# MyrtleSoftware/myrtlespeech

Measured on AMD Instinct MI355X. Metric: audio-sec/s (RTF), DS2 5xBiLSTM-1024 encoder forward + CTC greedy, 80-feature 10 s clips @ batch 32/GPU, higher is better.
Workload: dtype f16x3 (f32 split in fp16 hi+lo, 3 fp16 MFMA passes, f32 acc: LSTM, projections, conv1/2, FC1; FC2/CTC/decode f32)

## Files before the change

include/ms_hotpath.h:

```cpp
#ifndef MS_HOTPATH_H
#define MS_HOTPATH_H

#include <stddef.h>
#include <stdint.h>

#ifdef __cplusplus
extern "C" {
#endif

#define MS_ABI_VERSION 4

enum {
  MS_OK = 0,
  MS_ERR_INVALID = 1,
  MS_ERR_HIP = 2,
  MS_ERR_WORKSPACE = 3,
  MS_ERR_TIMEOUT = 4,
  MS_ERR_UNSUPPORTED = 5
};

enum { MS_CELL_LSTM = 0, MS_CELL_GRU = 1, MS_CELL_RNN_TANH = 2, MS_CELL_HARD_LSTM = 3 };

enum { MS_ACT_NONE = 0, MS_ACT_CLAMP = 1  };

int ms_abi_version(void);
const char* ms_last_error(void);


int ms_mask_time_(float* x, const int32_t* lens, int N, int inner, int T, void* stream);

size_t ms_maskconv_packed_bytes(int Cout, int Cin_g, int KF, int KT, int groups);

int ms_maskconv_pack(const float* w, void* packed, int Cout, int Cin_g, int KF, int KT, int groups, void* stream);

int ms_maskconv_forward(const float* x, const int32_t* lens, const void* packed_w, const float* bias, float* y,
                        int N, int Cin, int Fin, int Tin, int Cout, int Fout, int Tout, int KF, int KT, int SF,
                        int ST, int DF, int DT, int pad_f_l, int pad_t_l, int groups, int act, float act_lo,
                        float act_hi, void* stream);

size_t ms_maskconv_cl_packed_bytes(int Cout, int Cin, int KF, int KT);
int ms_maskconv_cl_pack(const float* w, void* packed, int Cout, int Cin, int KF, int KT, void* stream);
size_t ms_maskconv_cl_workspace_bytes(int N, int Cin, int Fin, int Tin);
int ms_maskconv_cl_forward(const float* x, const int32_t* lens, const void* packed_w, const float* bias, float* y,
                           int N, int Cin, int Fin, int Tin, int Cout, int Fout, int Tout, int KF, int KT, int SF,
                           int ST, int DF, int DT, int pad_f_l, int pad_t_l, int act, float act_lo, float act_hi,
                           void* workspace, size_t workspace_bytes, void* stream);

size_t ms_maskconv_fwin_packed_bytes(int Cout, int KF, int KT);
int ms_maskconv_fwin_pack(const float* w, void* packed, int Cout, int KF, int KT, void* stream);
size_t ms_maskconv_fwin_workspace_bytes(int N, int Tin, int KF, int SF, int Fout);
int ms_maskconv_fwin_forward(const float* x, const int32_t* lens, const void* packed_w, const float* bias, float* y, int N,
                             int Fin, int Tin, int Cout, int Fout, int Tout, int KF, int KT, int SF, int ST, int DT,
                             int pad_f_l, int pad_t_l, int act, float act_lo, float act_hi, void* workspace,
                             size_t workspace_bytes, void* stream);

int ms_maskconv_fwin_planes_supported(int N, int Tin, int Cout, int Fout, int Tout, int KF, int KT, int SF, int ST, int DT);
int ms_maskconv_cl_supported(int N, int Cin, int Fin, int Cout, int Fout, int Tout, int KT, int ST, int DT);
int ms_maskconv_fwin_planes_forward(const float* x, const int32_t* lens, const void* packed_w, const float* bias, void* planes,
                                    size_t planes_bytes, int N, int Fin, int Tin, int Cout, int Fout, int Tout, int KF, int KT,
                                    int SF, int ST, int DT, int pad_f_l, int pad_t_l, int act, float act_lo, float act_hi,
                                    void* workspace, size_t workspace_bytes, void* stream);
int ms_maskconv_cl_planes_forward(const int32_t* lens, const void* packed_w, const float* bias, float* y, int N, int Cin,
                                  int Fin, int Tin, int Cout, int Fout, int Tout, int KF, int KT, int SF, int ST, int DF,
                                  int DT, int pad_f_l, int pad_t_l, int act, float act_lo, float act_hi, void* planes,
                                  size_t planes_bytes, void* stream);

int ms_conv_set_variant(int variant);

size_t ms_maskconv1d_gemm_packed_bytes(int Cout, int Cin, int KT);
int ms_maskconv1d_gemm_pack(const float* w, void* packed, int Cout, int Cin, int KT, void* stream);
size_t ms_maskconv1d_gemm_workspace_bytes(int N, int Cin, int Tout, int Cout, int KT);
int ms_maskconv1d_gemm_forward(const float* x, const int32_t* lens, const void* packed, const float* bias, float* y, int N,
                               int Cin, int Tin, int Cout, int Tout, int KT, int ST, int DT, int pad_l, int act,
                               float act_lo, float act_hi, void* workspace, size_t workspace_bytes, void* stream);

int ms_nct_to_tnc(const float* x, float* y, int N, int CF, int T, void* stream);

int ms_clamp(const float* x, float* y, size_t n, float lo, float hi, void* stream);


int ms_linear_forward(const float* x, const float* w, const float* bias, float* y, int M, int K, int N, int act,
                      float act_lo, float act_hi, void* stream);

#define MS_LINEAR_FEW_ROWS 1
size_t ms_linear_splitk_workspace_bytes(int M, int K, int N, int flags);
int ms_linear_splitk_forward(const float* x, const float* w, const float* bias, float* y, int M, int K, int N, int act,
                             float act_lo, float act_hi, int flags, void* workspace, size_t workspace_bytes, void* stream);

size_t ms_linear_split_workspace_bytes(int M, int K, int N);
int ms_linear_split_forward(const float* x, const float* w, const float* bias, float* y, int M, int K, int N, int act,
                            float act_lo, float act_hi, void* workspace, size_t workspace_bytes, void* stream);

size_t ms_linear_split_packed_bytes(int K, int N);
int ms_linear_split_pack(const float* w, void* packed, int K, int N, void* stream);
int ms_linear_split_forward_packed(const float* x, const void* packed_w, const float* bias, float* y, int M, int K, int N, int act,
                                   float act_lo, float act_hi, void* workspace, size_t workspace_bytes, void* stream);


int ms_lookahead_forward(const float* x, const float* w, float* y, int N, int F, int T, int ctx, long xs_n,
                         long xs_f, long xs_t, long ys_n, long ys_f, long ys_t, int act, float act_lo,
                         float act_hi, void* stream);

int ms_lookahead_window_forward(const float* x, const float* w, float* y, int N, int F, int T_in, int T_out, int ctx,
                                long xs_n, long xs_f, long xs_t, long ys_n, long ys_f, long ys_t, int act, float act_lo,
                                float act_hi, void* stream);


int ms_rnn_padded_hidden(int cell, int H, int ndir);
size_t ms_rnn_packed_bytes(int cell, int In, int H, int ndir);
int ms_rnn_pack(int cell, int In, int H, int ndir, const float* const* w_ih_host, const float* const* w_hh_host,
                const float* const* b_ih_host, const float* const* b_hh_host, void* packed, void* stream);

size_t ms_rnn_workspace_bytes(int cell, int T, int N, int In, int H, int ndir);

int ms_rnn_layer_forward(int cell, const void* packed, const float* x, const int32_t* lens, int max_len,
                         const float* h0, const float* c0, float* out, float* hn, float* cn, int T, int N, int In,
                         int H, int ndir, void* workspace, size_t workspace_bytes, void* stream);

enum { MS_RNN_X_PLANES_IN_WS = 1, MS_RNN_OUT_PLANES_TO_WS = 2, MS_RNN_PACKED_ROWS = 4, MS_RNN_HX_PREINIT = 4096,
       MS_RNN_RECURRENCE_ONLY = 8192, MS_RNN_TIMING_SKIP_PROJECTION = 8192 ,
// ... 258 lines not shown
```

myrtlespeech_amd/_lib.py:

```python
import ctypes
import os
import re
from ctypes import POINTER, c_char_p, c_double, c_float, c_int, c_int32, c_int64, c_long, c_size_t, c_uint64, c_void_p

import torch

_HERE = os.path.dirname(os.path.abspath(__file__))
LIB_PATH = os.environ.get("MS_HOTPATH_LIB") or os.path.join(_HERE, "libms_hotpath.so")
HEADER_PATH = os.path.join(os.path.dirname(_HERE), "include", "ms_hotpath.h")

MS_OK = 0
ABI_VERSION = 4
ERR_NAMES = {1: "MS_ERR_INVALID", 2: "MS_ERR_HIP", 3: "MS_ERR_WORKSPACE", 4: "MS_ERR_TIMEOUT", 5: "MS_ERR_UNSUPPORTED"}

CELL_LSTM, CELL_GRU, CELL_RNN_TANH, CELL_HARD_LSTM = 0, 1, 2, 3
ACT_NONE, ACT_CLAMP = 0, 1
LINEAR_FEW_ROWS = 1
PROF_KINDS = 9

_P = c_void_p
_PP = POINTER(c_void_p)

SIGNATURES = {
    "ms_abi_version": (c_int, []),
    "ms_last_error": (c_char_p, []),
    "ms_mask_time_": (c_int, [_P, _P, c_int, c_int, c_int, _P]),
    "ms_maskconv_packed_bytes": (c_size_t, [c_int, c_int, c_int, c_int, c_int]),
    "ms_maskconv_pack": (c_int, [_P, _P, c_int, c_int, c_int, c_int, c_int, _P]),
    "ms_maskconv_forward": (c_int, [_P, _P, _P, _P, _P] + [c_int] * 17 + [c_float, c_float, _P]),
    "ms_maskconv_cl_packed_bytes": (c_size_t, [c_int, c_int, c_int, c_int]),
    "ms_maskconv_cl_pack": (c_int, [_P, _P, c_int, c_int, c_int, c_int, _P]),
    "ms_maskconv_cl_workspace_bytes": (c_size_t, [c_int, c_int, c_int, c_int]),
    "ms_maskconv_cl_forward": (c_int, [_P, _P, _P, _P, _P] + [c_int] * 16 + [c_float, c_float, _P, c_size_t, _P]),
    "ms_maskconv_fwin_packed_bytes": (c_size_t, [c_int, c_int, c_int]),
    "ms_maskconv_fwin_pack": (c_int, [_P, _P, c_int, c_int, c_int, _P]),
    "ms_maskconv_fwin_workspace_bytes": (c_size_t, [c_int, c_int, c_int, c_int, c_int]),
    "ms_maskconv_fwin_forward": (c_int, [_P, _P, _P, _P, _P] + [c_int] * 14 + [c_float, c_float, _P, c_size_t, _P]),
    "ms_maskconv_fwin_planes_forward": (c_int, [_P, _P, _P, _P, _P, c_size_t] + [c_int] * 14 + [c_float, c_float, _P, c_size_t, _P]),
    "ms_maskconv_cl_planes_forward": (c_int, [_P, _P, _P, _P] + [c_int] * 16 + [c_float, c_float, _P, c_size_t, _P]),
    "ms_maskconv_fwin_planes_supported": (c_int, [c_int] * 10),
    "ms_maskconv_cl_supported": (c_int, [c_int] * 9),
    "ms_conv_set_variant": (c_int, [c_int]),
    "ms_maskconv1d_gemm_packed_bytes": (c_size_t, [c_int, c_int, c_int]),
    "ms_maskconv1d_gemm_pack": (c_int, [_P, _P, c_int, c_int, c_int, _P]),
    "ms_maskconv1d_gemm_workspace_bytes": (c_size_t, [c_int] * 5),
    "ms_maskconv1d_gemm_forward": (c_int, [_P, _P, _P, _P, _P] + [c_int] * 10 + [c_float, c_float, _P, c_size_t, _P]),
    "ms_nct_to_tnc": (c_int, [_P, _P, c_int, c_int, c_int, _P]),
    "ms_clamp": (c_int, [_P, _P, c_size_t, c_float, c_float, _P]),
    "ms_linear_forward": (c_int, [_P, _P, _P, _P, c_int, c_int, c_int, c_int, c_float, c_float, _P]),
    "ms_linear_splitk_workspace_bytes": (c_size_t, [c_int, c_int, c_int, c_int]),
    "ms_linear_splitk_forward": (c_int, [_P, _P, _P, _P, c_int, c_int, c_int, c_int, c_float, c_float, c_int, _P, c_size_t, _P]),
    "ms_linear_split_workspace_bytes": (c_size_t, [c_int, c_int, c_int]),
    "ms_linear_split_forward": (c_int, [_P, _P, _P, _P, c_int, c_int, c_int, c_int, c_float, c_float, _P, c_size_t, _P]),
    "ms_linear_split_packed_bytes": (c_size_t, [c_int, c_int]),
    "ms_linear_split_pack": (c_int, [_P, _P, c_int, c_int, _P]),
    "ms_linear_split_forward_packed": (c_int, [_P, _P, _P, _P, c_int, c_int, c_int, c_int, c_float, c_float, _P, c_size_t, _P]),
    "ms_lookahead_forward": (c_int, [_P, _P, _P, c_int, c_int, c_int, c_int] + [c_long] * 6 + [c_int, c_float, c_float, _P]),
    "ms_lookahead_window_forward": (c_int, [_P, _P, _P, c_int, c_int, c_int, c_int, c_int] + [c_long] * 6 + [c_int, c_float, c_float, _P]),
    "ms_rnn_packed_bytes": (c_size_t, [c_int, c_int, c_int, c_int]),
    "ms_ctc_status": (c_int, [_P, _P]),
    "ms_rnn_padded_hidden": (c_int, [c_int, c_int, c_int]),
    "ms_rnn_hx_preinit": (c_int, [c_int] * 8 + [_P, c_size_t, _P]),
    "ms_rnn_pack": (c_int, [c_int, c_int, c_int, c_int, _PP, _PP, _PP, _PP, _P, _P]),
    "ms_rnn_workspace_bytes": (c_size_t, [c_int] * 6),
    "ms_rnn_layer_forward": (c_int, [c_int, _P, _P, _P, c_int, _P, _P, _P, _P, _P] + [c_int] * 5 + [_P, c_size_t, _P]),
    "ms_rnn_layer_forward_ex": (c_int, [c_int, _P, _P, _P, c_int, _P, _P, _P, _P, _P] + [c_int] * 6 + [_P, c_size_t, _P]),
    "ms_rnn_layer_chains_planes": (c_int, [c_int, c_int, c_int]),
    "ms_rnn_layer_is_wide": (c_int, [c_int] * 4),
    "ms_rnn_stack_overlap_ok": (c_int, [c_int] * 7),
    "ms_rnn_stack_forward": (c_int, [c_int, _P, _P, _P, c_int, _P, _P, _P, _P, _P] + [c_int] * 7 + [_P, c_size_t, _P]),
    "ms_rnn_status": (c_int, [_P, _P]),
    "ms_rnn_debug_offset": (c_size_t, [c_int] * 6),
    "ms_rnn_layer_packs_rows": (c_int, [c_int] * 6),
    "ms_gemm_set_variant": (c_int, [c_int]),
    "ms_prof_enable": (c_int, [c_int]),
    "ms_prof_read": (c_int, [POINTER(c_float), POINTER(c_int)]),
    "ms_clock_probe": (c_int, [_P, c_int, c_int, _P]),
    "ms_barrier_chain_probe": (c_int, [_P, c_int, c_int, _P]),
    "ms_ctc_loss_workspace_bytes": (c_size_t, [c_int] * 4),
    "ms_ctc_loss_forward": (c_int, [_P] * 7 + [c_int] * 7 + [_P, c_size_t, _P]),
    "ms_log_softmax_axis": (c_int, [_P, _P, c_int, c_int, c_int, _P]),
    "ms_log_softmax_axis_backward": (c_int, [_P, _P, _P, c_int, c_int, c_int, _P]),
    "ms_ctc_loss_backward_workspace_bytes": (c_size_t, [c_int] * 4),
    "ms_ctc_loss_backward": (c_int, [_P] * 7 + [c_int] * 6 + [_P, c_size_t, _P]),
    "ms_ctc_greedy_decode": (c_int, [_P, _P, _P, _P, c_int, c_int, c_int, c_int, _P]),
    "ms_ctc_align_workspace_bytes": (c_size_t, [c_int] * 4),
    "ms_ctc_align": (c_int, [_P] * 10 + [c_int] * 6 + [_P, c_size_t, _P]),
    "ms_ctc_greedy_stream_state_bytes": (c_size_t, [c_int]),
    "ms_ctc_greedy_stream_begin": (c_int, [_P, c_int, _P]),
    "ms_ctc_greedy_stream_step": (c_int, [_P, c_int, c_int, c_int, c_int, _P, _P, _P, _P, c_int, _P, _P, c_int, _P]),
    "ms_embedding_forward": (c_int, [_P, _P, _P, c_int, c_int, c_int, _P]),
    "ms_rnnt_joint_forward": (c_int, [_P, _P, _P, _P, _P, _P, c_int, c_int, c_int, _P]),
    "ms_rnnt_topk": (c_int, [_P, _P, _P, c_int, c_int, c_int, _P]),
    "ms_ctc_beam_workspace_bytes": (c_size_t, [c_int] * 4),
# ... 266 lines not shown
```

myrtlespeech_amd/csrc/api_common.cpp:

```cpp
#include <cstdlib>
#include <cstring>
#include <mutex>
#include <vector>

#include <algorithm>
#include "common.h"

namespace ms {
static thread_local std::string g_err;
void set_error(const std::string& s) { g_err = s; }
int num_cus() {
  static std::atomic<int> cus[64];
  int dev = 0;
  if (hipGetDevice(&dev) != hipSuccess) return 0;
  int v = cus[dev & 63].load(std::memory_order_relaxed);
  if (v == 0) {
    hipDeviceProp_t p;
    if (hipGetDeviceProperties(&p, dev) != hipSuccess) return 0;
    v = p.multiProcessorCount;
    cus[dev & 63].store(v, std::memory_order_relaxed);
  }
  return v;
}
int precision_mode() {
  static int v = -1;
  if (v < 0) {
    const char* e = getenv("MS_PRECISION");
    v = PREC_F16X3;
    if (e && strcmp(e, "f32") == 0) v = PREC_F32;
    if (e && strcmp(e, "fp16") == 0) v = PREC_F16;
    if (e && strcmp(e, "bf16x3") == 0) v = PREC_BF16X3;
  }
  return v;
}

namespace {
__global__ void absmax_bits_kernel(const float* __restrict__ w, size_t n, unsigned* __restrict__ out) {
  unsigned m = 0;
  for (size_t i = (size_t)blockIdx.x * blockDim.x + threadIdx.x; i < n; i += (size_t)gridDim.x * blockDim.x) {
    const unsigned b = __float_as_uint(w[i]) & 0x7FFFFFFFu;
    if (b < 0x7F800000u) m = max(m, b);
  }
  for (int o = 32; o > 0; o >>= 1) m = max(m, (unsigned)__shfl_xor((int)m, o, 64));
  if ((threadIdx.x & 63) == 0 && m) atomicMax(out, m);
}
__global__ void scale_word_kernel(float* __restrict__ word, int half_planes) {
  const unsigned bits = __float_as_uint(word[0]);
  int s = 0;
  if (half_planes && bits != 0) {
    const int e = (int)((bits >> 23) & 255) - 127;
    s = min(max(12 - e, -100), 100);
  }
  word[0] = ldexpf(1.0f, s);
  word[1] = ldexpf(1.0f, -s);
}
}

int weight_scale_launch(const float* w, size_t n, float* scale_word, int prec, hipStream_t stream) {
  MS_HIP(hipMemsetAsync(scale_word, 0, 2 * sizeof(float), stream));
  const bool half_planes = prec == PREC_F16X3 || prec == PREC_F16;
  if (half_planes && n > 0) {
    const int blocks = (int)std::min<size_t>((n + 255) / 256, 1024);
    hipLaunchKernelGGL(absmax_bits_kernel, dim3(blocks), dim3(256), 0, stream, w, n, (unsigned*)scale_word);
  }
  hipLaunchKernelGGL(scale_word_kernel, dim3(1), dim3(1), 0, stream, scale_word, half_planes ? 1 : 0);
  MS_LAUNCH_CHECK();
  return MS_OK;
}

namespace {
struct ProfSpan { hipEvent_t a, b; int kind; };
std::atomic<bool> g_prof_on{false};
std::mutex g_prof_mu;
std::vector<ProfSpan> g_spans;
std::vector<ProfSpan> g_free;
}

ProfScope::ProfScope(int kind_, hipStream_t st) : kind(kind_), stream(st), on(g_prof_on.load(std::memory_order_relaxed)) {
  if (!on) return;
  {
    std::lock_guard<std::mutex> lk(g_prof_mu);
    if (!g_free.empty()) { a = g_free.back().a; b = g_free.back().b; g_free.pop_back(); }
  }
  if (!a && (hipEventCreate(&a) != hipSuccess || hipEventCreate(&b) != hipSuccess)) { on = false; return; }
  (void)hipEventRecord(a, stream);
}
ProfScope::~ProfScope() {
  if (!on) return;
  (void)hipEventRecord(b, stream);
  std::lock_guard<std::mutex> lk(g_prof_mu);
  g_spans.push_back({a, b, kind});
}
}

extern "C" int ms_prof_enable(int on) {
  ms::g_prof_on.store(on != 0, std::memory_order_relaxed);
  return MS_OK;
}

extern "C" int ms_prof_read(float* out_ms, int* out_n) {
  MS_REQUIRE(out_ms && out_n, "null pointer");
  for (int k = 0; k < MS_PROF_KINDS; ++k) { out_ms[k] = 0.f; out_n[k] = 0; }
  std::lock_guard<std::mutex> lk(ms::g_prof_mu);
  for (auto& s : ms::g_spans) {
    MS_HIP(hipEventSynchronize(s.b));
    float t = 0.f;
    MS_HIP(hipEventElapsedTime(&t, s.a, s.b));
    if (s.kind >= 0 && s.kind < MS_PROF_KINDS) { out_ms[s.kind] += t; out_n[s.kind] += 1; }
    ms::g_free.push_back(s);
  }
  ms::g_spans.clear();
  return MS_OK;
}

// ... 57 lines not shown
```

myrtlespeech_amd/csrc/conv_cl.hip:

```cpp
#include <algorithm>
#include <type_traits>

#include "common.h"

namespace {

typedef unsigned u32x4 __attribute__((ext_vector_type(4)));
typedef unsigned u32x2 __attribute__((ext_vector_type(2)));
typedef __bf16 bf16x8 __attribute__((ext_vector_type(8)));
typedef _Float16 f16x8 __attribute__((ext_vector_type(8)));

constexpr int CL_F = 2;

struct ClP {
  int N, Cin, Fin, Tin, Cout, Fout, Tout, KF, KT, SF, ST, DF, DT, pad_f, pad_t;
  int KG;
  int KW;
  int PW;
  int co_tiles;
  int act;
  float lo, hi;
  int FP;
  int CS, RG, SG, PQ;
};
// ... 256 lines not shown
  };
  constexpr std::integral_constant<int, 0> S0{};
  constexpr std::integral_constant<int, 1> S1{};
  if (wave < p.KF) load_row(S0, wave);
  for (int kf = wave; kf < p.KF; kf += 8) {
    if (kf + 4 < p.KF) load_row(S1, kf + 4);
    compute_row(S0, kf);
    if (kf + 8 < p.KF) load_row(S0, kf + 8);
    if (kf + 4 < p.KF) compute_row(S1, kf + 4);
  }

  __syncthreads();
  ms::f32x4* part = reinterpret_cast<ms::f32x4*>(lds);
#pragma unroll
  for (int i = 0; i < SH_RB; ++i)
    if (i < RB) part[(wave * SH_RB + i) * 64 + lane] = acc[i];
  __syncthreads();
#pragma unroll
  for (int j = 0; j < SH_RB / 4; ++j) {
    const int i = wave + 4 * j, fo = fo0 + i;
    if (i >= RB || fo >= p.Fout) continue;
    ms::f32x4 v = part[(0 * SH_RB + i) * 64 + lane];
#pragma unroll
    for (int w = 1; w < 4; ++w) v += part[(w * SH_RB + i) * 64 + lane];
    if (c16 < p.Tout) {
#pragma unroll
      for (int r = 0; r < 4; ++r) {
        const int co = cb * 16 + 4 * q + r;
        if (co < p.Cout) {
          float o = v[r] * winv + (bias ? bias[co] : 0.f);
          if (p.act == MS_ACT_CLAMP) o = ms::act_clamp(o, p.lo, p.hi);
          y[(((size_t)n * p.Cout + co) * p.Fout + fo) * p.Tout + c16] = o;
        }
      }
    }
  }
}

int conv_cl_short_plan(const ClP& p, bool f16, int* RB, int* RIN, size_t* lds) {
  static const bool off = getenv("MS_CONV_SHORT") && getenv("MS_CONV_SHORT")[0] == '0';
  if (off || p.Cin != 32 || p.Tout > 16 || p.ST != 1 || p.DT != 1 || p.FP != 0 || p.N > 65535 || p.KT > SH_KT) return 0;
  const int cbs = ms::cdiv(p.Cout, 16);
  int nblk = std::max(1, std::min(ms::cdiv(p.Fout, 4), ms::cdiv(ms::num_cus(), p.N * cbs)));
  while (ms::cdiv(p.Fout, nblk) > SH_RB) ++nblk;
  for (; nblk <= p.Fout; ++nblk) {
    const int rb = ms::cdiv(p.Fout, nblk);
    const int rin = (rb - 1) * p.SF + (p.KF - 1) * p.DF + 1;
    const size_t bytes = std::max((size_t)(f16 ? 1 : 2) * rin * (p.Tout + p.KT - 1) * 64, (size_t)4 * SH_RB * 64 * 16);
    if (bytes <= 156 * 1024) { *RB = rb; *RIN = rin; *lds = bytes; return 1; }
  }
  return 0;
}

constexpr int FS_TT = 64;
constexpr int FS_MR = 5;
constexpr int FS_TS = 2;
constexpr int FS_PF = 2;

template <int P>
__global__ __launch_bounds__(256, 2) void maskconv_fwin_shared_kernel(const unsigned short* __restrict__ xh,
                                                                      const unsigned short* __restrict__ xl,
                                                                      const int32_t* __restrict__ lens,
                                                                      const unsigned short* __restrict__ wp,
                                                                      const float* __restrict__ bias, float* __restrict__ y,
                                                                      unsigned short* __restrict__ oh,
                                                                      unsigned short* __restrict__ ol, ClP p,
                                                                      const float* __restrict__ scale_word) {
  constexpr bool F16 = ms::prec_one_plane(P), HM = P == ms::PREC_F16X3;
  extern __shared__ __attribute__((aligned(16))) char lds[];
  const int gran_bytes = p.ST * p.PQ * 16;
  const int in_plane = p.SG * gran_bytes;
  char* Ph = lds;
  char* Pl = lds + in_plane;
  char* Wh = lds + (F16 ? 1 : 2) * in_plane;
  char* Wl = Wh + FS_TS * p.KG * 32 * 16;

  const int tid = threadIdx.x, lane = tid & 63, wave = tid >> 6;
  const int l31 = lane & 31, half = lane >> 5;
  const int fb = wave & 1, rg = wave >> 1;
  const int t0 = blockIdx.x * FS_TT;
  const int cls = blockIdx.y % p.CS, jb = blockIdx.y / p.CS;
  const int fo_first = cls + jb * (2 * FS_MR) * p.CS;
  if (fo_first >= p.Fout) return;
  const int nrows = min(2 * FS_MR, (p.Fout - 1 - fo_first) / p.CS + 1);
  const int n = blockIdx.z / p.co_tiles, tile = blockIdx.z % p.co_tiles;
  const int len = lens ? min(lens[n], p.Tin) : p.Tin;
  const int cout_pad = p.co_tiles * 32;
  const size_t wplane = (size_t)p.KT * p.KG * cout_pad * 8;

  u32x4 fh[FS_PF], fl[FS_PF];
  auto load_filters = [&](int kt0) {
    const int ng = min(FS_TS, p.KT - kt0) * p.KG * 32;
#pragma unroll
    for (int j = 0; j < FS_PF; ++j) {
      const int i = tid + 256 * j;
      if (i < ng) {
        const int co = i & 31, rest = i >> 5;
        const size_t src = (((size_t)kt0 * p.KG + rest) * cout_pad + tile * 32 + co) * 8;
        fh[j] = *reinterpret_cast<const u32x4*>(wp + src);
        if (!F16) fl[j] = *reinterpret_cast<const u32x4*>(wp + wplane + src);
      }
    }
  };
  auto store_filters = [&](int kt0) {
    const int ng = min(FS_TS, p.KT - kt0) * p.KG * 32;
#pragma unroll
// ... 74 lines not shown
          }
        }
      };
      for (int s = 0; s < s_full; ++s) k_step(s, std::false_type{});
      if (s_full < p.KG / 2) k_step(s_full, std::true_type{});
    }
    if (more) {
      __syncthreads();
      store_filters(kt0 + FS_TS);
      __syncthreads();
    }
  }

  const int t = t0 + fb * 32 + l31;
  const float winv = scale_word[1];
  if (t < p.Tout) {
#pragma unroll
    for (int f = 0; f < FS_MR; ++f) {
      const int j = rg * FS_MR + f;
      if (j >= nrows) continue;
      const int fo = fo_first + j * p.CS;
      if (oh) {
#pragma unroll
        for (int r4 = 0; r4 < 4; ++r4) {
          const int co = tile * 32 + ms::mfma32_row(4 * r4, lane);
          if (co >= p.Cout) continue;
          unsigned h[4], l[4];
#pragma unroll
          for (int e = 0; e < 4; ++e) {
            float v = acc[f][4 * r4 + e] * winv + (bias ? bias[co + e] : 0.f);
            if (p.act == MS_ACT_CLAMP) v = ms::act_clamp(v, p.lo, p.hi);
            split_act_by_prec(v, P, h[e], l[e]);
          }
          const size_t o = (((size_t)n * p.Fout + fo) * p.Tout + t) * p.Cout + co;
          *reinterpret_cast<u32x2*>(oh + o) = u32x2{h[0] | (h[1] << 16), h[2] | (h[3] << 16)};
          if (!F16) *reinterpret_cast<u32x2*>(ol + o) = u32x2{l[0] | (l[1] << 16), l[2] | (l[3] << 16)};
        }
        continue;
      }
#pragma unroll
      for (int r = 0; r < 16; ++r) {
        const int co = tile * 32 + ms::mfma32_row(r, lane);
        if (co < p.Cout) {
          float v = acc[f][r] * winv + (bias ? bias[co] : 0.f);
          if (p.act == MS_ACT_CLAMP) v = ms::act_clamp(v, p.lo, p.hi);
          y[(((size_t)n * p.Cout + co) * p.Fout + fo) * p.Tout + t] = v;
        }
      }
    }
  }
}

int conv_fs_plan(ClP& p, bool f16, size_t* lds) {
  if (g_conv_variant.load(std::memory_order_relaxed) != 0 || p.Tout <= 48 || p.SF % 2) return 0;
  int g = 2 * p.SF, b = 16;
  while (b) { const int r = g % b; g = b; b = r; }
  p.CS = 16 / g;
  p.RG = p.CS * p.SF / 8;
  p.SG = (2 * FS_MR - 1) * p.RG + p.KG;
  p.PW = (FS_TT - 1) * p.ST + (p.KT - 1) * p.DT + 1;
  p.PQ = ms::cdiv(p.PW, p.ST);
  const int planes = f16 ? 1 : 2;
  *lds = (size_t)planes * ((size_t)p.SG * p.ST * p.PQ * 16 + (size_t)FS_TS * p.KG * 32 * 16);
  const long rows_y = (long)p.CS * ms::cdiv(ms::cdiv(p.Fout, p.CS), 2 * FS_MR);
  if (p.SG > 16 || FS_TS * p.KG * 32 > 256 * FS_PF || *lds > 160 * 1024 || rows_y > 65535 || (long)p.N * p.co_tiles > 65535)
    return 0;
  return 1;
}

int conv_fs_launch(const ClP& p, size_t lds, const unsigned short* xh, const unsigned short* xl, const int32_t* lens,
                   const void* packed_w, const float* bias, float* y, unsigned short* oh, unsigned short* ol,
                   hipStream_t stream, const float* scale_word) {
  static ms::DeviceOnce attr_once;
  if (attr_once.need()) {
    MS_HIP(hipFuncSetAttribute((const void*)maskconv_fwin_shared_kernel<ms::PREC_BF16X3>, hipFuncAttributeMaxDynamicSharedMemorySize, 160 * 1024));
    MS_HIP(hipFuncSetAttribute((const void*)maskconv_fwin_shared_kernel<ms::PREC_F16>, hipFuncAttributeMaxDynamicSharedMemorySize, 160 * 1024));
    MS_HIP(hipFuncSetAttribute((const void*)maskconv_fwin_shared_kernel<ms::PREC_F16X3>, hipFuncAttributeMaxDynamicSharedMemorySize, 160 * 1024));
    attr_once.done();
  }
  const int prec = ms::split_mode();
  const dim3 grid(ms::cdiv(p.Tout, FS_TT), p.CS * ms::cdiv(ms::cdiv(p.Fout, p.CS), 2 * FS_MR), p.N * p.co_tiles);
  const unsigned short* wq = (const unsigned short*)packed_w;
  auto kern = prec == ms::PREC_F16 ? maskconv_fwin_shared_kernel<ms::PREC_F16>
              : prec == ms::PREC_F16X3 ? maskconv_fwin_shared_kernel<ms::PREC_F16X3> : maskconv_fwin_shared_kernel<ms::PREC_BF16X3>;
  hipLaunchKernelGGL(kern, grid, dim3(256), lds, stream, xh, xl, lens, wq, bias, y, oh, ol, p, scale_word);
  MS_LAUNCH_CHECK();
  return MS_OK;
}

__global__ void nchw_to_cl_split_kernel(const float* __restrict__ x, unsigned short* __restrict__ hi,
                                        unsigned short* __restrict__ lo, int C, int F, int T, int prec) {
  __shared__ float tile[32][33];
  const int n = blockIdx.z / F, f = blockIdx.z % F;
  const int t0 = blockIdx.x * 32, c0 = blockIdx.y * 32;
  const int tx = threadIdx.x, ty = threadIdx.y;
  for (int i = ty; i < 32; i += 8) {
    const int c = c0 + i, t = t0 + tx;
    tile[i][tx] = (c < C && t < T) ? x[(((size_t)n * C + c) * F + f) * T + t] : 0.f;
  }
  __syncthreads();
  for (int i = ty; i < 32; i += 8) {
    const int t = t0 + i, c = c0 + tx;
    if (t < T && c < C) {
      const float v = tile[tx][i];
      const size_t o = (((size_t)n * F + f) * T + t) * C + c;
      unsigned h, l;
      split_act_by_prec(v, prec, h, l);
// ... 201 lines not shown
  MS_REQUIRE(planes, "null pointer");
  MS_REQUIRE(Cout > 0 && Cout % 16 == 0, "planes out need Cout % 16 == 0 (the next convolution's k-steps)");
  if (N <= 0 || Fout <= 0 || Tout <= 0 || planes_bytes < ms_maskconv_cl_workspace_bytes(N, Cout, Fout, Tout)) {
    ms::set_error("ms_maskconv_fwin_planes_forward: planes buffer too small");
    return MS_ERR_WORKSPACE;
  }
  return fwin_forward(x, lens, packed_w, bias, nullptr, planes, N, Fin, Tin, Cout, Fout, Tout, KF, KT, SF, ST, DT, pad_f_l,
                      pad_t_l, act, act_lo, act_hi, workspace, workspace_bytes, stream_);
}

extern "C" int ms_conv_set_variant(int v) {
  g_conv_variant.store(v, std::memory_order_relaxed);
  return MS_OK;
}

static size_t cl_plane_bytes(int Cout, int Cin, int KF, int KT) {
  return ms::align_up((size_t)2 * KF * KT * (Cin / 8) * (ms::cdiv(Cout, 32) * 32) * 8 * sizeof(unsigned short), 256);
}
extern "C" size_t ms_maskconv_cl_packed_bytes(int Cout, int Cin, int KF, int KT) {
  if (Cout <= 0 || Cin <= 0 || Cin % 16 || KF <= 0 || KT <= 0) return 0;
  return cl_plane_bytes(Cout, Cin, KF, KT) + 256;
}

extern "C" int ms_maskconv_cl_pack(const float* w, void* packed, int Cout, int Cin, int KF, int KT, void* stream) {
  MS_REQUIRE(w && packed, "null pointer");
  MS_REQUIRE(Cout > 0 && Cin > 0 && Cin % 16 == 0 && KF > 0 && KT > 0, "bad shape (Cin must be a multiple of 16)");
  const int cout_pad = ms::cdiv(Cout, 32) * 32;
  const size_t plane = (size_t)KF * KT * (Cin / 8) * cout_pad * 8;
  const int blocks = (int)std::min<size_t>((plane + 255) / 256, 2048);
  float* scale_word = (float*)((char*)packed + cl_plane_bytes(Cout, Cin, KF, KT));
  const int rc = ms::weight_scale_launch(w, (size_t)Cout * Cin * KF * KT, scale_word, ms::split_mode(), (hipStream_t)stream);
  if (rc != MS_OK) return rc;
  hipLaunchKernelGGL(conv_cl_pack_kernel, dim3(blocks), dim3(256), 0, (hipStream_t)stream, w, (unsigned short*)packed, Cout,
                     Cin, KF, KT, cout_pad, ms::split_mode(), scale_word);
  MS_LAUNCH_CHECK();
  return MS_OK;
}

extern "C" size_t ms_maskconv_cl_workspace_bytes(int N, int Cin, int Fin, int Tin) {
  if (N <= 0 || Cin <= 0 || Fin <= 0 || Tin <= 0) return 0;
  return ms::align_up((size_t)N * Cin * Fin * Tin * 4, 256);
}

extern "C" int ms_maskconv_cl_supported(int N, int Cin, int Fin, int Cout, int Fout, int Tout, int KT, int ST, int DT) {
  if (N <= 0 || Cin <= 0 || Cin % 16 || Fin <= 0 || Cout <= 0 || Fout <= 0 || Tout <= 0 || KT <= 0 || ST <= 0 || DT <= 0 ||
      (long)N * Fin > 65535)
    return 0;
  ClP p{};
  p.N = N; p.Fout = Fout; p.Tout = Tout; p.KT = KT; p.ST = ST; p.DT = DT; p.KG = Cin / 8; p.co_tiles = ms::cdiv(Cout, 32);
  size_t lds = 0;
  return conv_cl_plan(p, &lds) != 0;
}

static int cl_forward(const float* x, const int32_t* lens, const void* packed_w, const float* bias, float* y,
                      int N, int Cin, int Fin, int Tin, int Cout, int Fout, int Tout, int KF, int KT,
                      int SF, int ST, int DF, int DT, int pad_f_l, int pad_t_l, int act, float act_lo,
                      float act_hi, void* workspace, size_t workspace_bytes, void* stream_) {
  ms::ProfScope prof_span(MS_PROF_CONV, (hipStream_t)stream_);
  MS_REQUIRE(packed_w && y && workspace, "null pointer");
  MS_REQUIRE(N > 0 && Cin > 0 && Cin % 16 == 0 && Fin > 0 && Tin > 0 && Cout > 0 && Fout > 0 && Tout > 0, "bad shape");
  MS_REQUIRE(KF > 0 && KT > 0 && SF > 0 && ST > 0 && DF > 0 && DT > 0 && pad_f_l >= 0 && pad_t_l >= 0, "bad kernel");
  MS_REQUIRE(act == MS_ACT_NONE || act == MS_ACT_CLAMP, "bad act");
  if (workspace_bytes < ms_maskconv_cl_workspace_bytes(N, Cin, Fin, Tin)) {
    ms::set_error("ms_maskconv_cl_forward: workspace too small");
    return MS_ERR_WORKSPACE;
  }
  hipStream_t stream = (hipStream_t)stream_;
  ClP p;
  p.N = N; p.Cin = Cin; p.Fin = Fin; p.Tin = Tin; p.Cout = Cout; p.Fout = Fout; p.Tout = Tout; p.KF = KF; p.KT = KT;
  p.SF = SF; p.ST = ST; p.DF = DF; p.DT = DT; p.pad_f = pad_f_l; p.pad_t = pad_t_l; p.KG = Cin / 8;
  p.co_tiles = ms::cdiv(Cout, 32);
  p.act = act; p.lo = act_lo; p.hi = act_hi;
  p.FP = 0;
  p.KW = 0;
  p.CS = p.RG = p.SG = p.PQ = 0;
  size_t lds = 0;
  const int wf = conv_cl_plan(p, &lds);
  if (wf == 0) {
    ms::set_error("ms_maskconv_cl_forward: shape outside the LDS / grid budget");
    return MS_ERR_UNSUPPORTED;
  }
  const float* scale_word = (const float*)((const char*)packed_w + cl_plane_bytes(Cout, Cin, KF, KT));
  unsigned short* xh = (unsigned short*)workspace;
  unsigned short* xl = xh + (size_t)N * Cin * Fin * Tin;
  MS_REQUIRE(N * Fin <= 65535, "N*Fin exceeds grid limits");
  const int prec = ms::split_mode();
  const bool f16 = prec == ms::PREC_F16;
  if (x) {
    hipLaunchKernelGGL(nchw_to_cl_split_kernel, dim3(ms::cdiv(Tin, 32), ms::cdiv(Cin, 32), N * Fin), dim3(32, 8), 0, stream, x,
                       xh, xl, Cin, Fin, Tin, prec);
    MS_LAUNCH_CHECK();
  }
  {
    int RB = 0, RIN = 0;
    size_t slds = 0;
    if (conv_cl_short_plan(p, f16, &RB, &RIN, &slds)) {
      static ms::DeviceOnce attr_once;
      if (attr_once.need()) {
        MS_HIP(hipFuncSetAttribute((const void*)maskconv_cl_short_kernel<ms::PREC_BF16X3>, hipFuncAttributeMaxDynamicSharedMemorySize, 160 * 1024));
        MS_HIP(hipFuncSetAttribute((const void*)maskconv_cl_short_kernel<ms::PREC_F16>, hipFuncAttributeMaxDynamicSharedMemorySize, 160 * 1024));
        MS_HIP(hipFuncSetAttribute((const void*)maskconv_cl_short_kernel<ms::PREC_F16X3>, hipFuncAttributeMaxDynamicSharedMemorySize, 160 * 1024));
        attr_once.done();
      }
      ClP ps = p;
      ps.PW = Tout + KT - 1;
      const dim3 grid(ms::cdiv(Fout, RB), ms::cdiv(Cout, 16), N);
      const unsigned short* wq = (const unsigned short*)packed_w;
      auto kern = prec == ms::PREC_F16 ? maskconv_cl_short_kernel<ms::PREC_F16>
                  : prec == ms::PREC_F16X3 ? maskconv_cl_short_kernel<ms::PREC_F16X3> : maskconv_cl_short_kernel<ms::PREC_BF16X3>;
      hipLaunchKernelGGL(kern, grid, dim3(256), slds, stream, xh, xl, lens, wq, bias, y, ps, RB, RIN, scale_word);
      MS_LAUNCH_CHECK();
      return MS_OK;
    }
  }
  return conv_cl_launch<false>(p, wf, lds, xh, xl, lens, packed_w, bias, y, stream, scale_word);
}

extern "C" int ms_maskconv_cl_forward(const float* x, const int32_t* lens, const void* packed_w, const float* bias, float* y,
                                      int N, int Cin, int Fin, int Tin, int Cout, int Fout, int Tout, int KF, int KT,
                                      int SF, int ST, int DF, int DT, int pad_f_l, int pad_t_l, int act, float act_lo,
                                      float act_hi, void* workspace, size_t workspace_bytes, void* stream_) {
  MS_REQUIRE(x, "null pointer");
  return cl_forward(x, lens, packed_w, bias, y, N, Cin, Fin, Tin, Cout, Fout, Tout, KF, KT, SF, ST, DF, DT, pad_f_l, pad_t_l,
                    act, act_lo, act_hi, workspace, workspace_bytes, stream_);
}

extern "C" int ms_maskconv_cl_planes_forward(const int32_t* lens, const void* packed_w, const float* bias, float* y, int N,
                                             int Cin, int Fin, int Tin, int Cout, int Fout, int Tout, int KF, int KT, int SF,
                                             int ST, int DF, int DT, int pad_f_l, int pad_t_l, int act, float act_lo,
                                             float act_hi, void* planes, size_t planes_bytes, void* stream_) {
  return cl_forward(nullptr, lens, packed_w, bias, y, N, Cin, Fin, Tin, Cout, Fout, Tout, KF, KT, SF, ST, DF, DT, pad_f_l,
                    pad_t_l, act, act_lo, act_hi, planes, planes_bytes, stream_);
}
```

Baseline: 28300.

## Add row-ring conv kernel streaming input frequency rows with double-buffered filters

Adds a new channels-last masked conv kernel that keeps a small ring of SF+1 input frequency rows in LDS and streams filter taps through double-buffered LDS stages, computing two output rows per block. Each loaded input row is reused across adjacent output rows instead of being re-staged per window. It is meant to cut redundant global-to-LDS traffic and LDS footprint for conv2. The weight absmax pass now also flags non-finite or near-max weights so padding-row skipping is only used when the weights are finite. The fs plan's variant gating also changes.

```diff
diff --git a/include/ms_hotpath.h b/include/ms_hotpath.h
--- a/include/ms_hotpath.h
+++ b/include/ms_hotpath.h
@@ -66,6 +66,8 @@
                                   size_t planes_bytes, void* stream);
 
 int ms_conv_set_variant(int variant);
+int ms_maskconv_cl_rows_supported(int N, int Cin, int Fin, int Cout, int Fout, int Tout, int KF, int KT, int SF, int ST, int DF,
+                                  int DT);
 
 size_t ms_maskconv1d_gemm_packed_bytes(int Cout, int Cin, int KT);
 int ms_maskconv1d_gemm_pack(const float* w, void* packed, int Cout, int Cin, int KT, void* stream);
diff --git a/myrtlespeech_amd/_lib.py b/myrtlespeech_amd/_lib.py
--- a/myrtlespeech_amd/_lib.py
+++ b/myrtlespeech_amd/_lib.py
@@ -40,6 +40,7 @@
     "ms_maskconv_cl_planes_forward": (c_int, [_P, _P, _P, _P] + [c_int] * 16 + [c_float, c_float, _P, c_size_t, _P]),
     "ms_maskconv_fwin_planes_supported": (c_int, [c_int] * 10),
     "ms_maskconv_cl_supported": (c_int, [c_int] * 9),
+    "ms_maskconv_cl_rows_supported": (c_int, [c_int] * 12),
     "ms_conv_set_variant": (c_int, [c_int]),
     "ms_maskconv1d_gemm_packed_bytes": (c_size_t, [c_int, c_int, c_int]),
     "ms_maskconv1d_gemm_pack": (c_int, [_P, _P, c_int, c_int, c_int, _P]),
diff --git a/myrtlespeech_amd/csrc/api_common.cpp b/myrtlespeech_amd/csrc/api_common.cpp
--- a/myrtlespeech_amd/csrc/api_common.cpp
+++ b/myrtlespeech_amd/csrc/api_common.cpp
@@ -36,16 +36,19 @@
 
 namespace {
 __global__ void absmax_bits_kernel(const float* __restrict__ w, size_t n, unsigned* __restrict__ out) {
-  unsigned m = 0;
+  unsigned m = 0, wild = 0;
   for (size_t i = (size_t)blockIdx.x * blockDim.x + threadIdx.x; i < n; i += (size_t)gridDim.x * blockDim.x) {
     const unsigned b = __float_as_uint(w[i]) & 0x7FFFFFFFu;
     if (b < 0x7F800000u) m = max(m, b);
+    if (b >= 0x7F7F8000u) wild = 1u;
   }
   for (int o = 32; o > 0; o >>= 1) m = max(m, (unsigned)__shfl_xor((int)m, o, 64));
   if ((threadIdx.x & 63) == 0 && m) atomicMax(out, m);
+  if (wild) atomicOr(out + 2, 1u);
 }
 __global__ void scale_word_kernel(float* __restrict__ word, int half_planes) {
   const unsigned bits = __float_as_uint(word[0]);
+  word[2] = __float_as_uint(word[2]) == 0u ? 1.0f : 0.0f;
   int s = 0;
   if (half_planes && bits != 0) {
     const int e = (int)((bits >> 23) & 255) - 127;
@@ -57,9 +60,9 @@
 }
 
 int weight_scale_launch(const float* w, size_t n, float* scale_word, int prec, hipStream_t stream) {
-  MS_HIP(hipMemsetAsync(scale_word, 0, 2 * sizeof(float), stream));
+  MS_HIP(hipMemsetAsync(scale_word, 0, 3 * sizeof(float), stream));
   const bool half_planes = prec == PREC_F16X3 || prec == PREC_F16;
-  if (half_planes && n > 0) {
+  if (n > 0) {
     const int blocks = (int)std::min<size_t>((n + 255) / 256, 1024);
     hipLaunchKernelGGL(absmax_bits_kernel, dim3(blocks), dim3(256), 0, stream, w, n, (unsigned*)scale_word);
   }
diff --git a/myrtlespeech_amd/csrc/conv_cl.hip b/myrtlespeech_amd/csrc/conv_cl.hip
--- a/myrtlespeech_amd/csrc/conv_cl.hip
+++ b/myrtlespeech_amd/csrc/conv_cl.hip
@@ -332,6 +332,272 @@
   return 0;
 }
 
+constexpr int RW_RPT = 4;
+constexpr int RW_FPT = 3;
+
+template <int P>
+__global__ __launch_bounds__(256, 2) __attribute__((amdgpu_waves_per_eu(2, 2))) void maskconv_cl_rows_kernel(const unsigned short* __restrict__ xh,
+                                                                  const unsigned short* __restrict__ xl,
+                                                                  const int32_t* __restrict__ lens,
+                                                                  const unsigned short* __restrict__ wp,
+                                                                  const float* __restrict__ bias, float* __restrict__ y, ClP p,
+                                                                  int TS, const float* __restrict__ scale_word) {
+  constexpr bool F16 = ms::prec_one_plane(P), HM = P == ms::PREC_F16X3;
+  constexpr int NP = F16 ? 1 : 2;
+  extern __shared__ __attribute__((aligned(16))) char lds[];
+  const int R = p.SF + 1;
+  const int row_bytes = p.KG * p.PW * 16;
+  const int slot_bytes = NP * row_bytes;
+  const int wtap = p.KG * 32 * 16;
+  const int wbuf_bytes = NP * TS * wtap;
+  char* Wbase = lds + R * slot_bytes;
+
+  const int tid = threadIdx.x, lane = tid & 63, wave = __builtin_amdgcn_readfirstlane(tid >> 6);
+  const int l31 = lane & 31, half = lane >> 5;
+  const int t0 = blockIdx.x * 128;
+  const int fo0 = blockIdx.y * CL_F;
+  const int n = blockIdx.z / p.co_tiles, tile = blockIdx.z % p.co_tiles;
+  const int len = lens ? min(lens[n], p.Tin) : p.Tin;
+  const int cout_pad = p.co_tiles * 32;
+  const size_t wplane = (size_t)p.KF * p.KT * p.KG * cout_pad * 8;
+  const bool finite = scale_word[2] == 1.0f;
+  const bool wave_live = t0 + wave * 32 < p.Tout;
+  const int nfr = min(128, (p.Tout - t0 + 31) / 32 * 32);
+  const int ngran = p.KG * ((nfr - 1) * p.ST + (p.KT - 1) * p.DT + 1);
+  const int tin0 = t0 * p.ST - p.pad_t;
+  const int base = fo0 * p.SF - p.pad_f;
+
+  int ka[CL_F], kb[CL_F], kfa = p.KF, kfb = -1;
+#pragma unroll
+  for (int f = 0; f < CL_F; ++f) {
+    const int b = base + f * p.SF;
+    ka[f] = finite ? max(0, -b) : 0;
+    kb[f] = finite ? min(p.KF - 1, p.Fin - 1 - b) : p.KF - 1;
+    if (fo0 + f >= p.Fout) { ka[f] = p.KF; kb[f] = -1; }
+    if (ka[f] <= kb[f]) { kfa = min(kfa, ka[f]); kfb = max(kfb, kb[f]); }
+  }
+
+  ms::f32x16 acc[CL_F];
+#pragma unroll
+  for (int f = 0; f < CL_F; ++f)
+#pragma unroll
+    for (int r = 0; r < 16; ++r) acc[f][r] = 0.f;
+
+  struct RowRegs { u32x4 h[RW_RPT], l[RW_RPT]; };
+  RowRegs rr;
+  u32x4 fh[RW_FPT], fl[RW_FPT];
+  auto load_row = [&](RowRegs& g, int j) {
+    const int fin = base + j;
+    const bool in = fin >= 0 && fin < p.Fin;
+    const size_t rbase = ((size_t)n * p.Fin + (in ? fin : 0)) * p.Tin;
+#pragma unroll
+    for (int k = 0; k < RW_RPT; ++k) {
+      const int i = tid + 256 * k;
+      g.h[k] = u32x4{0u, 0u, 0u, 0u};
+      if constexpr (!F16) g.l[k] = u32x4{0u, 0u, 0u, 0u};
+      if (in && i < ngran) {
+        const int q = i / p.KG, kg = i - q * p.KG;
+        const int tin = tin0 + q;
+        if (tin >= 0 && tin < len) {
+          const size_t off = (rbase + tin) * p.Cin + kg * 8;
+          g.h[k] = *reinterpret_cast<const u32x4*>(xh + off);
+          if constexpr (!F16) g.l[k] = *reinterpret_cast<const u32x4*>(xl + off);
+        }
+      }
+    }
+  };
+  auto store_row = [&](const RowRegs& g, int j) {
+    const int fin = base + j;
+    if (finite && (fin < 0 || fin >= p.Fin)) return;
+    char* dst = lds + (j % R) * slot_bytes;
+#pragma unroll
+    for (int k = 0; k < RW_RPT; ++k) {
+      const int i = tid + 256 * k;
+      if (i < ngran) {
+        const int q = i / p.KG, kg = i - q * p.KG;
+        *reinterpret_cast<u32x4*>(dst + (kg * p.PW + q) * 16) = g.h[k];
+        if constexpr (!F16) *reinterpret_cast<u32x4*>(dst + row_bytes + (kg * p.PW + q) * 16) = g.l[k];
+      }
+    }
+  };
+  auto load_filters = [&](int kf, int kt0) {
+    const int ng = min(TS, p.KT - kt0) * p.KG * 32;
+#pragma unroll
+    for (int k = 0; k < RW_FPT; ++k) {
+      const int i = tid + 256 * k;
+      if (i < ng) {
+        const int co = i & 31, rest = i >> 5;
+        const size_t src = ((((size_t)kf * p.KT + kt0) * p.KG + rest) * cout_pad + tile * 32 + co) * 8;
+        fh[k] = *reinterpret_cast<const u32x4*>(wp + src);
+        if constexpr (!F16) fl[k] = *reinterpret_cast<const u32x4*>(wp + wplane + src);
+      }
+    }
+  };
+  auto store_filters = [&](int kt0, int buf) {
+    const int ng = min(TS, p.KT - kt0) * p.KG * 32;
+    char* Wh = Wbase + buf * wbuf_bytes;
+#pragma unroll
+    for (int k = 0; k < RW_FPT; ++k) {
+      const int i = tid + 256 * k;
+      if (i < ng) {
+        *reinterpret_cast<u32x4*>(Wh + i * 16) = fh[k];
+        if constexpr (!F16) *reinterpret_cast<u32x4*>(Wh + TS * wtap + i * 16) = fl[k];
+      }
+    }
+  };
+  struct Frag { u32x4 ah, al, bh[CL_F], bl[CL_F]; };
+  auto compute = [&](int kf, int kt0, int buf, auto mask) {
+    constexpr int MASK = decltype(mask)::value;
+    const char* Wh = Wbase + buf * wbuf_bytes;
+    const char* Wl = Wh + TS * wtap;
+    const int steps = min(TS, p.KT - kt0) * (p.KG / 2);
+    const char* rows[CL_F];
+#pragma unroll
+    for (int f = 0; f < CL_F; ++f) rows[f] = lds + ((f * p.SF + kf) % R) * slot_bytes;
+    int ktl = 0, s = 0;
+    auto fetch = [&](Frag& g) {
+      const int kg = 2 * s + half;
+      const int woff = ((ktl * p.KG + kg) * 32 + l31) * 16;
+      const int poff = (kg * p.PW + (wave * 32 + l31) * p.ST + (kt0 + ktl) * p.DT) * 16;
+      g.ah = *reinterpret_cast<const u32x4*>(Wh + woff);
+      if constexpr (!F16) g.al = *reinterpret_cast<const u32x4*>(Wl + woff);
+#pragma unroll
+      for (int f = 0; f < CL_F; ++f) {
+        if (!((MASK >> f) & 1)) continue;
+        g.bh[f] = *reinterpret_cast<const u32x4*>(rows[f] + poff);
+        if constexpr (!F16) g.bl[f] = *reinterpret_cast<const u32x4*>(rows[f] + row_bytes + poff);
+      }
+      if (++s == p.KG / 2) { s = 0; ++ktl; }
+    };
+    auto mfmas = [&](const Frag& g) {
+#pragma unroll
+      for (int f = 0; f < CL_F; ++f) {
+        if (!((MASK >> f) & 1)) continue;
+        if constexpr (F16) {
+          acc[f] = __builtin_amdgcn_mfma_f32_32x32x16_f16(__builtin_bit_cast(f16x8, g.ah), __builtin_bit_cast(f16x8, g.bh[f]), acc[f], 0, 0, 0);
+        } else {
+          acc[f] = ms::mfma_32x32x16<HM>(g.ah, g.bh[f], acc[f]);
+          acc[f] = ms::mfma_32x32x16<HM>(g.al, g.bh[f], acc[f]);
+          acc[f] = ms::mfma_32x32x16<HM>(g.ah, g.bl[f], acc[f]);
+        }
+      }
+    };
+    Frag a, b;
+    fetch(a);
+    int it = 0;
+    for (; it + 2 < steps; it += 2) {
+      fetch(b);
+      mfmas(a);
+      fetch(a);
+      mfmas(b);
+    }
+    if (it + 1 < steps) {
+      fetch(b);
+      mfmas(a);
+      mfmas(b);
+    } else {
+      mfmas(a);
+    }
+  };
+  static_assert(CL_F == 2, "the stage masks below name two output rows");
+
+  if (kfa <= kfb) {
+    {
+      RowRegs r1, r2;
+      load_filters(kfa, 0);
+      load_row(rr, kfa);
+      load_row(r1, kfa + 1);
+      if (p.SF == 2) load_row(r2, kfa + 2);
+      store_filters(0, 0);
+      store_row(rr, kfa);
+      store_row(r1, kfa + 1);
+      if (p.SF == 2) store_row(r2, kfa + 2);
+    }
+    int lkf = kfa, lkt = 0;
+    auto load_next_filters = [&]() {
+      lkt += TS;
+      if (lkt >= p.KT) { lkt = 0; ++lkf; }
+      if (lkf <= kfb) load_filters(lkf, lkt);
+    };
+    load_next_filters();
+    __syncthreads();
+    int buf = 0;
+    for (int kf = kfa; kf <= kfb; ++kf) {
+      const bool row_next = kf < kfb;
+      const int m = (kf >= ka[0] && kf <= kb[0] ? 1 : 0) | (kf >= ka[1] && kf <= kb[1] ? 2 : 0);
+      for (int kt0 = 0; kt0 < p.KT; kt0 += TS) {
+        const bool last = kt0 + TS >= p.KT;
+        const bool more = !last || row_next;
+        if (kt0 == 0 && row_next) load_row(rr, p.SF + kf + 1);
+        if (wave_live) {
+          if (m == 3) compute(kf, kt0, buf, std::integral_constant<int, 3>{});
+          else if (m == 1) compute(kf, kt0, buf, std::integral_constant<int, 1>{});
+          else if (m == 2) compute(kf, kt0, buf, std::integral_constant<int, 2>{});
+        }
+        if (last && row_next) {
+          __syncthreads();
+          store_row(rr, p.SF + kf + 1);
+        }
+        if (more) {
+          store_filters(lkt, buf ^ 1);
+          load_next_filters();
+          __syncthreads();
+        }
+        buf ^= 1;
+      }
+    }
+  }
+
+  const int t = t0 + wave * 32 + l31;
+  const float winv = scale_word[1];
+  if (t < p.Tout) {
+    float bv[16];
+#pragma unroll
+    for (int r = 0; r < 16; ++r) {
+      const int co = tile * 32 + ms::mfma32_row(r, lane);
+      bv[r] = bias && co < p.Cout ? bias[co] : 0.f;
+    }
+#pragma unroll
+    for (int f = 0; f < CL_F; ++f) {
+      const int fo = fo0 + f;
+      if (fo >= p.Fout) continue;
+#pragma unroll
+      for (int r = 0; r < 16; ++r) {
+        const int co = tile * 32 + ms::mfma32_row(r, lane);
+        if (co < p.Cout) {
+          float v = acc[f][r] * winv + bv[r];
+          if (p.act == MS_ACT_CLAMP) v = ms::act_clamp(v, p.lo, p.hi);
+          y[(((size_t)n * p.Cout + co) * p.Fout + fo) * p.Tout + t] = v;
+        }
+      }
+    }
+  }
+}
+
+int conv_cl_rows_plan(ClP& p, bool f16, int* TS, size_t* lds) {
+  static const int ts_env = getenv("MS_CONV_ROWS_TS") ? atoi(getenv("MS_CONV_ROWS_TS")) : 0;
+  if (g_conv_variant.load(std::memory_order_relaxed) != 0 || p.FP != 0 || p.DF != 1 || p.SF > 2) return 0;
+  if ((long)p.N * p.co_tiles > 65535 || ms::cdiv(p.Fout, CL_F) > 65535) return 0;
+  const int tt = std::min(128, ms::cdiv(p.Tout, 32) * 32);
+  const int pw = (tt - 1) * p.ST + (p.KT - 1) * p.DT + 1;
+  const int np = f16 ? 1 : 2;
+  const size_t ring = (size_t)(p.SF + 1) * np * p.KG * pw * 16;
+  const size_t wstage = (size_t)2 * np * p.KG * 32 * 16;
+  const int ts_max = std::min(p.KT, 8 * RW_FPT / p.KG);
+  if (p.KG * pw > 256 * RW_RPT || ts_max < 1) return 0;
+  int ts = 0;
+  for (size_t limit : {(size_t)80 * 1024, (size_t)160 * 1024}) {
+    if (ts == 0 && ring + wstage <= limit) ts = (int)std::min<size_t>(ts_max, (limit - ring) / wstage);
+  }
+  if (ts_env > 0 && ts_env <= ts_max && ring + ts_env * wstage <= (size_t)160 * 1024) ts = ts_env;
+  if (ts == 0) return 0;
+  ts = ms::cdiv(p.KT, ms::cdiv(p.KT, ts));
+  p.PW = pw;
+  *TS = ts;
+  *lds = ring + ts * wstage;
+  return 1;
+}
+
 constexpr int FS_TT = 64;
 constexpr int FS_MR = 5;
 constexpr int FS_TS = 2;
@@ -512,7 +778,7 @@
 }
 
 int conv_fs_plan(ClP& p, bool f16, size_t* lds) {
-  if (g_conv_variant.load(std::memory_order_relaxed) != 0 || p.Tout <= 48 || p.SF % 2) return 0;
+  if (g_conv_variant.load(std::memory_order_relaxed) == 1 || p.Tout <= 48 || p.SF % 2) return 0;
   int g = 2 * p.SF, b = 16;
   while (b) { const int r = g % b; g = b; b = r; }
   p.CS = 16 / g;
@@ -820,6 +1086,19 @@
   return conv_cl_plan(p, &lds) != 0;
 }
 
+extern "C" int ms_maskconv_cl_rows_supported(int N, int Cin, int Fin, int Cout, int Fout, int Tout, int KF, int KT, int SF, int ST,
+                                             int DF, int DT) {
+  if (KF <= 0 || SF <= 0 || DF <= 0 || !ms_maskconv_cl_supported(N, Cin, Fin, Cout, Fout, Tout, KT, ST, DT)) return 0;
+  ClP p{};
+  p.N = N; p.Cin = Cin; p.Fin = Fin; p.Cout = Cout; p.Fout = Fout; p.Tout = Tout; p.KF = KF; p.KT = KT; p.SF = SF; p.ST = ST;
+  p.DF = DF; p.DT = DT; p.KG = Cin / 8; p.co_tiles = ms::cdiv(Cout, 32);
+  const bool f16 = ms::split_mode() == ms::PREC_F16;
+  int RB = 0, RIN = 0, ts = 0;
+  size_t lds = 0;
+  if (conv_cl_short_plan(p, f16, &RB, &RIN, &lds)) return 0;
+  return conv_cl_rows_plan(p, f16, &ts, &lds);
+}
+
 static int cl_forward(const float* x, const int32_t* lens, const void* packed_w, const float* bias, float* y,
                       int N, int Cin, int Fin, int Tin, int Cout, int Fout, int Tout, int KF, int KT,
                       int SF, int ST, int DF, int DT, int pad_f_l, int pad_t_l, int act, float act_lo,
@@ -881,6 +1160,27 @@
       return MS_OK;
     }
   }
+  {
+    ClP pr = p;
+    int ts = 0;
+    size_t rlds = 0;
+    if (conv_cl_rows_plan(pr, f16, &ts, &rlds)) {
+      static ms::DeviceOnce attr_once;
+      if (attr_once.need()) {
+        MS_HIP(hipFuncSetAttribute((const void*)maskconv_cl_rows_kernel<ms::PREC_BF16X3>, hipFuncAttributeMaxDynamicSharedMemorySize, 160 * 1024));
+        MS_HIP(hipFuncSetAttribute((const void*)maskconv_cl_rows_kernel<ms::PREC_F16>, hipFuncAttributeMaxDynamicSharedMemorySize, 160 * 1024));
+        MS_HIP(hipFuncSetAttribute((const void*)maskconv_cl_rows_kernel<ms::PREC_F16X3>, hipFuncAttributeMaxDynamicSharedMemorySize, 160 * 1024));
+        attr_once.done();
+      }
+      const dim3 grid(ms::cdiv(Tout, 128), ms::cdiv(Fout, CL_F), N * p.co_tiles);
+      const unsigned short* wq = (const unsigned short*)packed_w;
+      auto kern = prec == ms::PREC_F16 ? maskconv_cl_rows_kernel<ms::PREC_F16>
+                  : prec == ms::PREC_F16X3 ? maskconv_cl_rows_kernel<ms::PREC_F16X3> : maskconv_cl_rows_kernel<ms::PREC_BF16X3>;
+      hipLaunchKernelGGL(kern, grid, dim3(256), rlds, stream, xh, xl, lens, wq, bias, y, pr, ts, scale_word);
+      MS_LAUNCH_CHECK();
+      return MS_OK;
+    }
+  }
   return conv_cl_launch<false>(p, wf, lds, xh, xl, lens, packed_w, bias, y, stream, scale_word);
 }
 
```

After: 28540 (median of 5 runs). About the same (+0.8%).
